# Guitaricet/relora

Hardware: NVIDIA H100
Metric: training throughput, llama ReLoRA (tokens/s, whole job, device-timed, max over ranks) (higher is better)
Workload: dtype bf16

## Files before the change

relora_b200/csrc/attention.cu:

```cuda
#include <cuda.h>

#include <cstdio>
#include <cstdlib>
#include <mutex>
#include <stdexcept>
#include <string>
#include <unordered_map>

#include "attention.h"
#include "common.cuh"
#include "sm90.cuh"
#include "tensormap.h"

namespace rb {

using namespace sm90;

namespace {

constexpr int BQ = 64;
constexpr int kPanel = 64 * 128;
constexpr int kThreads = 128;
constexpr int kMaxHeadDim = 256;
constexpr float kNegInf = -1e30f;

constexpr int smem_bytes(int nres, int np) { return (nres + 4) * np * kPanel + 1024 + 1024; }
constexpr int dq_out_panels(int np) { return np <= 3 ? np : 2; }
constexpr int dkv_out_panels(int np) { return np <= 2 ? np : 2; }
constexpr int splits(int np, int no) { return (np + no - 1) / no; }

__device__ __forceinline__ float fast_exp2(float x) {
  float y;
  asm("ex2.approx.ftz.f32 %0, %1;" : "=f"(y) : "f"(x));
  return y;
}

__device__ __forceinline__ void frag_to_a(const float (&d)[32], int kk, uint32_t (&a)[4]) {
  a[0] = pack_bf16x2(d[8 * kk + 0], d[8 * kk + 1]);
  a[1] = pack_bf16x2(d[8 * kk + 2], d[8 * kk + 3]);
  a[2] = pack_bf16x2(d[8 * kk + 4], d[8 * kk + 5]);
  a[3] = pack_bf16x2(d[8 * kk + 6], d[8 * kk + 7]);
}
template <int NSTEPS>
__device__ __forceinline__ void mma_steps_kk(float (&d)[32], uint32_t a, uint32_t b) {
#pragma unroll
  for (int ks = 0; ks < NSTEPS; ++ks) {
    const uint32_t ofs = (ks >> 2) * kPanel + (ks & 3) * 32;
    wgmma_bf16_ss_n64<0, 0>(d, desc_kmajor(a + ofs), desc_kmajor(b + ofs));
  }
}
template <int NP>
__device__ __forceinline__ void mma_tiles_kk(float (&d)[32], uint32_t a, uint32_t b, int nks) {
  if constexpr (NP == 1) {
    mma_steps_kk<4>(d, a, b);
  } else {
    switch (nks - 4 * (NP - 1)) {
      case 1: mma_steps_kk<4 * NP - 3>(d, a, b); break;
      case 2: mma_steps_kk<4 * NP - 2>(d, a, b); break;
      case 3: mma_steps_kk<4 * NP - 1>(d, a, b); break;
      default: mma_steps_kk<4 * NP>(d, a, b); break;
    }
  }
}
__device__ __forceinline__ void pack_a(const float (&p)[32], uint32_t (&a)[4][4]) {
#pragma unroll
  for (int kk = 0; kk < 4; ++kk) {
    frag_to_a(p, kk, a[kk]);
    fence_regs(a[kk]);
  }
}
template <int NO, int N = NO>
__device__ __forceinline__ void mma_regs_tile(float (&d)[NO][32], const uint32_t (&a)[4][4], uint32_t t, int nout) {
  if constexpr (N > 1) {
    if (nout < N) return mma_regs_tile<NO, N - 1>(d, a, t, nout);
  }
#pragma unroll
  for (int kk = 0; kk < 4; ++kk) {
#pragma unroll
    for (int j = 0; j < N; ++j) wgmma_bf16_rs_n64<1>(d[j], a[kk], desc_mnmajor(t + j * kPanel + kk * 2048));
  }
}
__device__ __forceinline__ void zero32(float (&d)[32]) {
#pragma unroll
  for (int i = 0; i < 32; ++i) d[i] = 0.f;
}

struct Smem {
  uint8_t* res[2];
  uint8_t* str[2][2];
  uint64_t* res_bar;
  uint64_t* str_bar;
  float* col_lse;
  float* col_delta;
};
template <int NRES, int NP>
__device__ __forceinline__ Smem smem_layout() {
  constexpr int kTile = NP * kPanel;
  extern __shared__ uint8_t smem_raw[];
  uint8_t* s = reinterpret_cast<uint8_t*>((reinterpret_cast<uintptr_t>(smem_raw) + 1023) & ~uintptr_t(1023));
  Smem m;
  m.res[0] = s;
  m.res[1] = s + (NRES - 1) * kTile;
  for (int b = 0; b < 2; ++b)
    for (int o = 0; o < 2; ++o) m.str[b][o] = s + (NRES + 2 * b + o) * kTile;
  m.res_bar = reinterpret_cast<uint64_t*>(s + (NRES + 4) * kTile);
  m.str_bar = m.res_bar + 1;
  m.col_lse = reinterpret_cast<float*>(s + (NRES + 4) * kTile + 64);
  m.col_delta = m.col_lse + 64;
  return m;
}
struct TileSrc {
  const CUtensorMap* map;
  int head;
};
template <int NP>
__device__ __forceinline__ void load_tile(TileSrc s, uint64_t* bar, uint8_t* dst, int row) {
#pragma unroll
  for (int pn = 0; pn < NP; ++pn) tma_load_3d(s.map, bar, dst + pn * kPanel, 64 * pn, s.head, row);
}
template <int NP>
__device__ __forceinline__ void issue_pair(const Smem& m, int buf, TileSrc s0, TileSrc s1, int row) {
  mbar_arrive_expect_tx(&m.str_bar[buf], 2 * NP * kPanel);
  load_tile<NP>(s0, &m.str_bar[buf], m.str[buf][0], row);
  load_tile<NP>(s1, &m.str_bar[buf], m.str[buf][1], row);
}
template <int NRES, int NP>
__device__ __forceinline__ void prologue(const Smem& m, TileSrc r0, TileSrc r1, int res_row, TileSrc s0, TileSrc s1, int row0, int nblk) {
  if (threadIdx.x == 0) {
    mbar_init(m.res_bar, 1);
    mbar_init(&m.str_bar[0], 1);
    mbar_init(&m.str_bar[1], 1);
    fence_barrier_init();
  }
  __syncthreads();
  pdl_wait();
  if (warp_id() == 0) {
    if (elect_one()) {
      mbar_arrive_expect_tx(m.res_bar, NRES * NP * kPanel);
      load_tile<NP>(r0, m.res_bar, m.res[0], res_row);
      if (NRES == 2) load_tile<NP>(r1, m.res_bar, m.res[1], res_row);
      for (int j = 0; j < 2 && j < nblk; ++j) issue_pair<NP>(m, j, s0, s1, row0 + j * BQ);
    }
    __syncwarp();
  }
  mbar_wait(m.res_bar, 0);
}

struct HeadMap {
  int hs, wk, wv, group;
  __device__ __forceinline__ int q(int h) const { return h * hs; }
  __device__ __forceinline__ int k(int kv) const { return kv * hs + wk; }
  __device__ __forceinline__ int v(int kv) const { return kv * hs + wv; }
};
struct FwdArgs {
  bf16* out;
  long long ld_out;
  float* lse;
  int B, T, nh, hd;
  float scale_log2;
  HeadMap hm;
};

template <int NP>
__global__ void __launch_bounds__(kThreads) attn_fwd_kernel(const __grid_constant__ CUtensorMap map_qkv, const FwdArgs p) {
  if (threadIdx.x == 0) pdl_launch_dependents();
  const int nqb = (p.T + BQ - 1) / BQ;
  const int qb = nqb - 1 - blockIdx.x;
  const int h = blockIdx.y, b = blockIdx.z;
  const int q0 = qb * BQ, rowbase = b * p.T;
  const int nkb = qb + 1;
  const int nks = (p.hd + 15) / 16;
  const Smem m = smem_layout<1, NP>();
  const int kv = h / p.hm.group;
  const int hq = p.hm.q(h), hk = p.hm.k(kv), hv = p.hm.v(kv);
  prologue<1, NP>(m, {&map_qkv, hq}, {&map_qkv, hq}, rowbase + q0, {&map_qkv, hk}, {&map_qkv, hv}, rowbase, nkb);
  const uint32_t sq = smem_u32(m.res[0]);
  float o[NP][32], mrow[2] = {kNegInf, kNegInf}, lrow[2] = {0.f, 0.f};
#pragma unroll
  for (int pn = 0; pn < NP; ++pn) zero32(o[pn]);
  const int r_lo = q0 + frag_row(0);
  for (int j = 0; j < nkb; ++j) {
    const int buf = j & 1;
    mbar_wait(&m.str_bar[buf], (j >> 1) & 1);
    float s[32];
    zero32(s);
    wgmma_fence();
    mma_tiles_kk<NP>(s, sq, smem_u32(m.str[buf][0]), nks);
    wgmma_commit();
    wgmma_wait<0>();
    fence_regs(s);
    float mx[2] = {mrow[0], mrow[1]};
#pragma unroll
    for (int i = 0; i < 32; ++i) {
      const int hr = (i >> 1) & 1;
      float v = s[i] * p.scale_log2;
      if (j == qb && j * BQ + frag_col(i) > r_lo + 8 * hr) v = kNegInf;
      s[i] = v;
      mx[hr] = fmaxf(mx[hr], v);
    }
#pragma unroll
    for (int hr = 0; hr < 2; ++hr) {
      mx[hr] = fmaxf(mx[hr], __shfl_xor_sync(0xffffffffu, mx[hr], 1));
      mx[hr] = fmaxf(mx[hr], __shfl_xor_sync(0xffffffffu, mx[hr], 2));
    }
    const float corr[2] = {fast_exp2(mrow[0] - mx[0]), fast_exp2(mrow[1] - mx[1])};
    float ls[2] = {0.f, 0.f};
#pragma unroll
    for (int i = 0; i < 32; ++i) {
      const int hr = (i >> 1) & 1;
      s[i] = fast_exp2(s[i] - mx[hr]);
      ls[hr] += s[i];
#pragma unroll
      for (int pn = 0; pn < NP; ++pn) o[pn][i] *= corr[hr];
    }
#pragma unroll
    for (int hr = 0; hr < 2; ++hr) {
      lrow[hr] = lrow[hr] * corr[hr] + ls[hr];
      mrow[hr] = mx[hr];
    }
    uint32_t pa[4][4];
    pack_a(s, pa);
#pragma unroll
    for (int pn = 0; pn < NP; ++pn) fence_regs(o[pn]);
    wgmma_fence();
    mma_regs_tile<NP>(o, pa, smem_u32(m.str[buf][1]), NP);
    wgmma_commit();
    wgmma_wait<0>();
#pragma unroll
    for (int pn = 0; pn < NP; ++pn) fence_regs(o[pn]);
    __syncthreads();
    if (warp_id() == 0 && j + 2 < nkb) {
      if (elect_one()) issue_pair<NP>(m, buf, {&map_qkv, hk}, {&map_qkv, hv}, rowbase + (j + 2) * BQ);
      __syncwarp();
    }
  }
#pragma unroll
  for (int hr = 0; hr < 2; ++hr) {
    lrow[hr] += __shfl_xor_sync(0xffffffffu, lrow[hr], 1);
    lrow[hr] += __shfl_xor_sync(0xffffffffu, lrow[hr], 2);
  }
#pragma unroll
  for (int pn = 0; pn < NP; ++pn) {
#pragma unroll
    for (int i = 0; i < 32; i += 2) {
      const int hr = (i >> 1) & 1;
      const int q = r_lo + 8 * hr, c = 64 * pn + frag_col(i);
      if (q >= p.T || c >= p.hd) continue;
      const float inv = 1.f / lrow[hr];
      *reinterpret_cast<uint32_t*>(p.out + (long long)(rowbase + q) * p.ld_out + h * p.hd + c) =
          pack_bf16x2(o[pn][i] * inv, o[pn][i + 1] * inv);
    }
  }
  if ((threadIdx.x & 3) == 0) {
#pragma unroll
    for (int hr = 0; hr < 2; ++hr) {
      const int q = r_lo + 8 * hr;
      if (q < p.T) p.lse[((long long)b * p.nh + h) * p.T + q] = mrow[hr] + __log2f(lrow[hr]);
    }
  }
}

__global__ void __launch_bounds__(256) attn_delta_kernel(const bf16* __restrict__ o, long long ld_o, const bf16* __restrict__ dout,
                                                         long long ld_do, float* __restrict__ delta, int B, int T, int nh, int hd) {
  pdl_wait();
  pdl_launch_dependents();
  const long long total = (long long)B * T * nh;
  for (long long i = blockIdx.x * (long long)blockDim.x + threadIdx.x; i < total; i += (long long)gridDim.x * blockDim.x) {
    const int h = int(i % nh);
    const long long row = i / nh;
    const bf16* a = o + row * ld_o + h * hd;
    const bf16* g = dout + row * ld_do + h * hd;
    float acc = 0.f;
    for (int q = 0; q < hd; q += 8) {
      float x[8], y[8];
      unpack8(*reinterpret_cast<const uint4*>(a + q), x);
      unpack8(*reinterpret_cast<const uint4*>(g + q), y);
#pragma unroll
      for (int j = 0; j < 8; ++j) acc += x[j] * y[j];
    }
    const long long bb = row / T, t = row % T;
    delta[(bb * nh + h) * T + t] = acc;
  }
}

struct BwdArgs {
  const float* lse;
  const float* delta;
  bf16* dqkv;
  long long ld_dqkv;
  int B, T, nh, hd;
  float scale, scale_log2;
  HeadMap hm;
};

__device__ __forceinline__ void store_rows(bf16* base, long long ld, int row0, int rows_valid, int col_ofs, int hd, const float (&d)[32], float sc) {
#pragma unroll
  for (int i = 0; i < 32; i += 2) {
    const int r = frag_row(i), c = frag_col(i);
    if (row0 + r >= rows_valid || c >= hd) continue;
    *reinterpret_cast<uint32_t*>(base + (long long)row0 * ld + (long long)r * ld + col_ofs + c) = pack_bf16x2(d[i] * sc, d[i + 1] * sc);
  }
}
template <int NO>
__device__ __forceinline__ void store_panels(bf16* base, long long ld, int row0, int rows_valid, int col_ofs, int hd, int pn0, int nout,
                                             const float (&d)[NO][32], float sc) {
#pragma unroll
  for (int j = 0; j < NO; ++j)
    if (j < nout) store_rows(base, ld, row0, rows_valid, col_ofs + 64 * (pn0 + j), hd - 64 * (pn0 + j), d[j], sc);
}

template <int NP>
__global__ void __launch_bounds__(kThreads) attn_bwd_dq_kernel(const __grid_constant__ CUtensorMap map_qkv,
                                                               const __grid_constant__ CUtensorMap map_do, const BwdArgs p) {
  constexpr int NO = dq_out_panels(NP), NSPLIT = splits(NP, dq_out_panels(NP));
  if (threadIdx.x == 0) pdl_launch_dependents();
  const int nqb = (p.T + BQ - 1) / BQ;
  const int qb = nqb - 1 - blockIdx.x / NSPLIT;
  const int pn0 = (blockIdx.x % NSPLIT) * NO;
  const int nout = NP % NO == 0 ? NO : min(NO, NP - pn0);
  const int h = blockIdx.y, b = blockIdx.z;
  const int q0 = qb * BQ, rowbase = b * p.T;
  const int nkb = qb + 1;
  const int nks = (p.hd + 15) / 16;
  const Smem m = smem_layout<2, NP>();
  const int kv = h / p.hm.group;
  const int hq = p.hm.q(h), hk = p.hm.k(kv), hv = p.hm.v(kv);
  prologue<2, NP>(m, {&map_qkv, hq}, {&map_do, h}, rowbase + q0, {&map_qkv, hk}, {&map_qkv, hv}, rowbase, nkb);
  const long long bh = (long long)b * p.nh + h;
  const int r_lo = q0 + frag_row(0);
  float lse[2], dlt[2];
#pragma unroll
  for (int hr = 0; hr < 2; ++hr) {
    const int q = min(r_lo + 8 * hr, p.T - 1);
    lse[hr] = p.lse[bh * p.T + q];
    dlt[hr] = p.delta[bh * p.T + q];
  }
  float dq[NO][32];
#pragma unroll
  for (int j = 0; j < NO; ++j) zero32(dq[j]);
  for (int j = 0; j < nkb; ++j) {
    const int buf = j & 1;
    mbar_wait(&m.str_bar[buf], (j >> 1) & 1);
    float s[32], dp[32];
    zero32(s);
    zero32(dp);
    wgmma_fence();
    mma_tiles_kk<NP>(s, smem_u32(m.res[0]), smem_u32(m.str[buf][0]), nks);
    mma_tiles_kk<NP>(dp, smem_u32(m.res[1]), smem_u32(m.str[buf][1]), nks);
    wgmma_commit();
    wgmma_wait<0>();
    fence_regs(s);
    fence_regs(dp);
#pragma unroll
    for (int i = 0; i < 32; ++i) {
      const int hr = (i >> 1) & 1;
      const bool ok = !(j == qb && j * BQ + frag_col(i) > r_lo + 8 * hr);
      const float pr = ok ? fast_exp2(s[i] * p.scale_log2 - lse[hr]) : 0.f;
      s[i] = pr * (dp[i] - dlt[hr]);
    }
    uint32_t pa[4][4];
    pack_a(s, pa);
    wgmma_fence();
    mma_regs_tile<NO>(dq, pa, smem_u32(m.str[buf][0]) + pn0 * kPanel, nout);
    wgmma_commit();
    wgmma_wait<0>();
#pragma unroll
    for (int jo = 0; jo < NO; ++jo) fence_regs(dq[jo]);
    __syncthreads();
    if (warp_id() == 0 && j + 2 < nkb) {
      if (elect_one()) issue_pair<NP>(m, buf, {&map_qkv, hk}, {&map_qkv, hv}, rowbase + (j + 2) * BQ);
      __syncwarp();
    }
  }
  store_panels<NO>(p.dqkv + (long long)rowbase * p.ld_dqkv, p.ld_dqkv, q0, p.T, hq * p.hd, p.hd, pn0, nout, dq, p.scale);
}

template <int NP>
__global__ void __launch_bounds__(kThreads) attn_bwd_dkv_kernel(const __grid_constant__ CUtensorMap map_qkv,
                                                                const __grid_constant__ CUtensorMap map_do, const BwdArgs p) {
  constexpr int NO = dkv_out_panels(NP), NSPLIT = splits(NP, dkv_out_panels(NP));
  if (threadIdx.x == 0) pdl_launch_dependents();
  const int nkb = (p.T + BQ - 1) / BQ;
  const int kb = blockIdx.x / NSPLIT;
  const int pn0 = (blockIdx.x % NSPLIT) * NO;
  const int nout = NP % NO == 0 ? NO : min(NO, NP - pn0);
  const int kv = blockIdx.y, b = blockIdx.z;
  const int k0 = kb * BQ, rowbase = b * p.T;
  const int nblk = nkb - kb;
  const int nks = (p.hd + 15) / 16;
  const Smem m = smem_layout<2, NP>();
  const int h0 = kv * p.hm.group;
  prologue<2, NP>(m, {&map_qkv, p.hm.k(kv)}, {&map_qkv, p.hm.v(kv)}, rowbase + k0, {&map_qkv, p.hm.q(h0)}, {&map_do, h0}, rowbase + k0, nblk);
  if (nblk == 1 && p.hm.group > 1 && warp_id() == 0) {
    if (elect_one()) issue_pair<NP>(m, 1, {&map_qkv, p.hm.q(h0 + 1)}, {&map_do, h0 + 1}, rowbase + k0);
    __syncwarp();
  }
  const int key_lo = k0 + frag_row(0);
  float dk[NO][32], dv[NO][32];
#pragma unroll
  for (int j = 0; j < NO; ++j) {
    zero32(dk[j]);
    zero32(dv[j]);
  }
  int hg = h0, qs = k0;
  for (int jj = 0; hg < ((int)blockIdx.y + 1) * p.hm.group; ++jj) {
    const int buf = jj & 1;
    const long long bh = (long long)b * p.nh + hg;
    if (threadIdx.x < BQ) {
      const int qc = min(qs + (int)threadIdx.x, p.T - 1);
      m.col_lse[threadIdx.x] = p.lse[bh * p.T + qc];
      m.col_delta[threadIdx.x] = p.delta[bh * p.T + qc];
    }
    __syncthreads();
    mbar_wait(&m.str_bar[buf], (jj >> 1) & 1);
    float st[32], dpt[32];
    zero32(st);
    zero32(dpt);
    wgmma_fence();
    mma_tiles_kk<NP>(st, smem_u32(m.res[0]), smem_u32(m.str[buf][0]), nks);
    mma_tiles_kk<NP>(dpt, smem_u32(m.res[1]), smem_u32(m.str[buf][1]), nks);
    wgmma_commit();
    wgmma_wait<0>();
    fence_regs(st);
    fence_regs(dpt);
#pragma unroll
    for (int i = 0; i < 32; ++i) {
      const int q = qs + frag_col(i), key = key_lo + 8 * ((i >> 1) & 1);
      const bool ok = q < p.T && key <= q;
      const float pr = ok ? fast_exp2(st[i] * p.scale_log2 - m.col_lse[frag_col(i)]) : 0.f;
      dpt[i] = pr * (dpt[i] - m.col_delta[frag_col(i)]);
      st[i] = pr;
    }
    uint32_t pa[4][4], dsa[4][4];
    pack_a(st, pa);
    pack_a(dpt, dsa);
    wgmma_fence();
    mma_regs_tile<NO>(dv, pa, smem_u32(m.str[buf][1]) + pn0 * kPanel, nout);
    mma_regs_tile<NO>(dk, dsa, smem_u32(m.str[buf][0]) + pn0 * kPanel, nout);
    wgmma_commit();
    wgmma_wait<0>();
#pragma unroll
    for (int j = 0; j < NO; ++j) {
      fence_regs(dv[j]);
      fence_regs(dk[j]);
    }
    __syncthreads();
    if (warp_id() == 0) {
      int h2 = hg, q2 = qs + 2 * BQ;
      while (q2 >= p.T) {
        q2 -= nkb * BQ - k0;
        ++h2;
      }
      if (h2 < ((int)blockIdx.y + 1) * p.hm.group) {
        if (elect_one()) issue_pair<NP>(m, buf, {&map_qkv, p.hm.q(h2)}, {&map_do, h2}, rowbase + q2);
        __syncwarp();
      }
    }
    qs += BQ;
    if (qs >= p.T) {
      qs = k0;
      ++hg;
    }
  }
  bf16* base = p.dqkv + (long long)rowbase * p.ld_dqkv;
  store_panels<NO>(base, p.ld_dqkv, k0, p.T, p.hm.k(blockIdx.y) * p.hd, p.hd, pn0, nout, dk, p.scale);
  store_panels<NO>(base, p.ld_dqkv, k0, p.T, p.hm.v(blockIdx.y) * p.hd, p.hd, pn0, nout, dv, 1.0f);
}

struct HeadMapKey {
  const void* ptr;
  long long ld, rows;
  int hd, heads;
  bool operator==(const HeadMapKey& o) const { return ptr == o.ptr && ld == o.ld && rows == o.rows && hd == o.hd && heads == o.heads; }
};
struct HeadMapHash {
  size_t operator()(const HeadMapKey& k) const {
    size_t h = reinterpret_cast<size_t>(k.ptr);
    h ^= std::hash<long long>()(k.ld * 1315423911ll + k.rows) + 0x9e3779b97f4a7c15ull + (h << 6) + (h >> 2);
    h ^= std::hash<long long>()(((long long)k.hd << 32) | (unsigned)k.heads) + 0x9e3779b97f4a7c15ull + (h << 6) + (h >> 2);
    return h;
  }
};
std::unordered_map<HeadMapKey, CUtensorMap, HeadMapHash> g_head_maps;
std::mutex g_head_maps_mu;

CUtensorMap head_map(const void* ptr, long long ld, long long rows, int hd, int heads) {
  HeadMapKey key{ptr, ld, rows, hd, heads};
  {
    std::lock_guard<std::mutex> lk(g_head_maps_mu);
    auto it = g_head_maps.find(key);
    if (it != g_head_maps.end()) return it->second;
  }
  CUtensorMap m = make_map_3d_bf16(ptr, hd, heads, rows, hd, ld, 64, 1, 64);
  std::lock_guard<std::mutex> lk(g_head_maps_mu);
  if (g_head_maps.size() > 4096) g_head_maps.clear();
  g_head_maps.emplace(key, m);
  return m;
}

void check_shape(int B, int T, int nh, int nkv, int hd, bool interleaved) {
  if (B <= 0 || T <= 0 || nh <= 0) throw std::runtime_error("attention: empty problem");
  if (hd <= 0 || hd % 8 != 0 || hd > kMaxHeadDim)
    throw std::runtime_error("attention: head_dim must be a multiple of 8 and <= 256, got " + std::to_string(hd));
  if (nkv <= 0 || nh % nkv != 0)
    throw std::runtime_error("attention: nh (" + std::to_string(nh) + ") must be a multiple of nkv (" + std::to_string(nkv) + ")");
  if (interleaved && nkv != nh) throw std::runtime_error("attention: the interleaved qkv layout has no grouped-query form (nkv must equal nh)");
}

HeadMap head_map_of(int nh, int nkv, bool interleaved) {
  return interleaved ? HeadMap{3, 1, 2, 1} : HeadMap{1, nh, nh + nkv, nh / nkv};
}

template <int NP>
void fwd_np(const AttnDesc& d, const CUtensorMap& map, cudaStream_t stream) {
  constexpr int smem = smem_bytes(1, NP);
  static const bool configured =
      (check(cudaFuncSetAttribute(attn_fwd_kernel<NP>, cudaFuncAttributeMaxDynamicSharedMemorySize, smem), "cudaFuncSetAttribute(attn_fwd)"), true);
  (void)configured;
  FwdArgs p;
  p.out = reinterpret_cast<bf16*>(d.out); p.ld_out = d.ld_out; p.lse = d.lse;
  p.B = d.B; p.T = d.T; p.nh = d.nh; p.hd = d.hd;
  p.scale_log2 = d.scale * 1.4426950408889634f;
  p.hm = head_map_of(d.nh, d.nkv, d.interleaved);
  const dim3 grid((unsigned)((d.T + BQ - 1) / BQ), (unsigned)d.nh, (unsigned)d.B);
  launch_k(attn_fwd_kernel<NP>, grid, kThreads, smem, stream, map, p);
  RB_CHECK_LAUNCH("attn_fwd_kernel");
}

template <int NP>
void bwd_np(const AttnBwdDesc& d, const CUtensorMap& map_qkv, const CUtensorMap& map_do, cudaStream_t stream) {
  constexpr int smem = smem_bytes(2, NP);
  static const bool configured =
      (check(cudaFuncSetAttribute(attn_bwd_dq_kernel<NP>, cudaFuncAttributeMaxDynamicSharedMemorySize, smem), "cudaFuncSetAttribute(attn_dq)"),
       check(cudaFuncSetAttribute(attn_bwd_dkv_kernel<NP>, cudaFuncAttributeMaxDynamicSharedMemorySize, smem), "cudaFuncSetAttribute(attn_dkv)"),
       true);
  (void)configured;
  BwdArgs p;
  p.lse = d.lse; p.delta = d.delta; p.dqkv = reinterpret_cast<bf16*>(d.dqkv); p.ld_dqkv = d.ld_dqkv;
  p.B = d.B; p.T = d.T; p.nh = d.nh; p.hd = d.hd;
  p.scale = d.scale; p.scale_log2 = d.scale * 1.4426950408889634f;
  p.hm = head_map_of(d.nh, d.nkv, d.interleaved);
  const unsigned nblk = (unsigned)((d.T + BQ - 1) / BQ);
  const dim3 grid_dkv(nblk * splits(NP, dkv_out_panels(NP)), (unsigned)d.nkv, (unsigned)d.B);
  launch_k(attn_bwd_dkv_kernel<NP>, grid_dkv, kThreads, smem, stream, map_qkv, map_do, p);
  RB_CHECK_LAUNCH("attn_bwd_dkv_kernel");
  const dim3 grid_dq(nblk * splits(NP, dq_out_panels(NP)), (unsigned)d.nh, (unsigned)d.B);
  launch_k(attn_bwd_dq_kernel<NP>, grid_dq, kThreads, smem, stream, map_qkv, map_do, p);
  RB_CHECK_LAUNCH("attn_bwd_dq_kernel");
}

int panels(int hd) { return (hd + 63) / 64; }

}

void attention_fwd(const AttnDesc& d, cudaStream_t stream) {
  check_shape(d.B, d.T, d.nh, d.nkv, d.hd, d.interleaved);
  const long long rows = (long long)d.B * d.T;
  CUtensorMap map = head_map(d.qkv, d.ld_qkv, rows, d.hd, d.nh + 2 * d.nkv);
  switch (panels(d.hd)) {
    case 1: fwd_np<1>(d, map, stream); break;
    case 2: fwd_np<2>(d, map, stream); break;
    case 3: fwd_np<3>(d, map, stream); break;
    default: fwd_np<4>(d, map, stream); break;
  }
}

void attention_bwd(const AttnBwdDesc& d, cudaStream_t stream) {
  check_shape(d.B, d.T, d.nh, d.nkv, d.hd, d.interleaved);
  const long long rows = (long long)d.B * d.T;
  CUtensorMap map_qkv = head_map(d.qkv, d.ld_qkv, rows, d.hd, d.nh + 2 * d.nkv);
  CUtensorMap map_do = head_map(d.dout, d.ld_dout, rows, d.hd, d.nh);
  {
    const long long total = rows * d.nh;
    const int grid = (int)std::min<long long>((total + 255) / 256, (long long)num_sms() * 8);
    launch_k(attn_delta_kernel, grid, 256, 0, stream, reinterpret_cast<const bf16*>(d.out), d.ld_out, reinterpret_cast<const bf16*>(d.dout),
             d.ld_dout, d.delta, d.B, d.T, d.nh, d.hd);
    RB_CHECK_LAUNCH("attn_delta_kernel");
  }
  switch (panels(d.hd)) {
    case 1: bwd_np<1>(d, map_qkv, map_do, stream); break;
    case 2: bwd_np<2>(d, map_qkv, map_do, stream); break;
    case 3: bwd_np<3>(d, map_qkv, map_do, stream); break;
    default: bwd_np<4>(d, map_qkv, map_do, stream); break;
  }
}

int attention_smem_bytes(int hd) { return smem_bytes(2, panels(hd)); }

long long attention_ds_pitch(int T) { return ((long long)T + 63) / 64 * 64; }
long long attention_ds_workspace_elems(int B, int T, int nh) {
  const long long Tp = attention_ds_pitch(T);
  return (long long)B * nh * Tp * Tp;
}

}
```

Before: 214,400.

## Coalesce delta kernel loads and overlap LSE/delta fetches with TMA waits

Rewrites the attention backward delta kernel so each warp cooperatively loads 32 (row, head) dot products with coalesced 16-byte loads, stages them in swizzled shared memory, and then has each lane reduce one row. The mbarrier wait on the resident Q/K/V tiles moves out of the prologue into each kernel, so LSE and delta loads overlap the TMA transfers. The dK/dV kernel also prefetches the next block's LSE/delta into registers during the current block. The delta path is a small share of the step, and the extra shared staging adds some complexity.

```diff
diff --git a/relora_b200/csrc/attention.cu b/relora_b200/csrc/attention.cu
--- a/relora_b200/csrc/attention.cu
+++ b/relora_b200/csrc/attention.cu
@@ -143,7 +143,6 @@
     }
     __syncwarp();
   }
-  mbar_wait(m.res_bar, 0);
 }
 
 struct HeadMap {
@@ -174,6 +173,7 @@
   const int kv = h / p.hm.group;
   const int hq = p.hm.q(h), hk = p.hm.k(kv), hv = p.hm.v(kv);
   prologue<1, NP>(m, {&map_qkv, hq}, {&map_qkv, hq}, rowbase + q0, {&map_qkv, hk}, {&map_qkv, hv}, rowbase, nkb);
+  mbar_wait(m.res_bar, 0);
   const uint32_t sq = smem_u32(m.res[0]);
   float o[NP][32], mrow[2] = {kNegInf, kNegInf}, lrow[2] = {0.f, 0.f};
 #pragma unroll
@@ -260,26 +260,57 @@
   }
 }
 
-__global__ void __launch_bounds__(256) attn_delta_kernel(const bf16* __restrict__ o, long long ld_o, const bf16* __restrict__ dout,
-                                                         long long ld_do, float* __restrict__ delta, int B, int T, int nh, int hd) {
+constexpr int kDeltaWarps = 4;
+constexpr int kDeltaChunks = 8;
+__global__ void __launch_bounds__(kDeltaWarps * 32) attn_delta_kernel(const bf16* __restrict__ o, long long ld_o, const bf16* __restrict__ dout,
+                                                                       long long ld_do, float* __restrict__ delta, int B, int T, int nh, int hd) {
+  __shared__ uint4 stage[kDeltaWarps][2][32][kDeltaChunks];
   pdl_wait();
   pdl_launch_dependents();
   const long long total = (long long)B * T * nh;
-  for (long long i = blockIdx.x * (long long)blockDim.x + threadIdx.x; i < total; i += (long long)gridDim.x * blockDim.x) {
-    const int h = int(i % nh);
-    const long long row = i / nh;
-    const bf16* a = o + row * ld_o + h * hd;
-    const bf16* g = dout + row * ld_do + h * hd;
+  const int lane = threadIdx.x & 31, w = threadIdx.x >> 5;
+  const int cpr = hd / 8;
+  for (long long s0 = ((long long)blockIdx.x * kDeltaWarps + w) * 32; s0 < total; s0 += (long long)gridDim.x * kDeltaWarps * 32) {
+    const long long row0 = s0 / nh;
+    const int h0 = int(s0 - row0 * nh);
     float acc = 0.f;
-    for (int q = 0; q < hd; q += 8) {
-      float x[8], y[8];
-      unpack8(*reinterpret_cast<const uint4*>(a + q), x);
-      unpack8(*reinterpret_cast<const uint4*>(g + q), y);
-#pragma unroll
-      for (int j = 0; j < 8; ++j) acc += x[j] * y[j];
-    }
-    const long long bb = row / T, t = row % T;
-    delta[(bb * nh + h) * T + t] = acc;
+    for (int c0 = 0; c0 < cpr; c0 += kDeltaChunks) {
+      const int nc = min(kDeltaChunks, cpr - c0);
+      uint4 xr[kDeltaChunks], yr[kDeltaChunks];
+#pragma unroll
+      for (int r = 0; r < kDeltaChunks; ++r) {
+        const int k = lane + 32 * r, ls = k / nc, c = k - ls * nc;
+        if (r < nc && s0 + ls < total) {
+          const int hh = h0 + ls;
+          const long long row = row0 + hh / nh;
+          const int col = (hh % nh) * hd + 8 * (c0 + c);
+          xr[r] = *reinterpret_cast<const uint4*>(o + row * ld_o + col);
+          yr[r] = *reinterpret_cast<const uint4*>(dout + row * ld_do + col);
+        }
+      }
+#pragma unroll
+      for (int r = 0; r < kDeltaChunks; ++r) {
+        const int k = lane + 32 * r, ls = k / nc, c = k - ls * nc;
+        if (r < nc && s0 + ls < total) {
+          stage[w][0][ls][c ^ (ls & 7)] = xr[r];
+          stage[w][1][ls][c ^ (ls & 7)] = yr[r];
+        }
+      }
+      __syncwarp();
+      for (int c = 0; c < nc; ++c) {
+        float x[8], y[8];
+        unpack8(stage[w][0][lane][c ^ (lane & 7)], x);
+        unpack8(stage[w][1][lane][c ^ (lane & 7)], y);
+#pragma unroll
+        for (int j = 0; j < 8; ++j) acc += x[j] * y[j];
+      }
+      __syncwarp();
+    }
+    if (s0 + lane < total) {
+      const int hh = h0 + lane;
+      const long long row = row0 + hh / nh, bb = row / T, t = row % T;
+      delta[(bb * nh + hh % nh) * T + t] = acc;
+    }
   }
 }
 
@@ -335,6 +366,7 @@
     lse[hr] = p.lse[bh * p.T + q];
     dlt[hr] = p.delta[bh * p.T + q];
   }
+  mbar_wait(m.res_bar, 0);
   float dq[NO][32];
 #pragma unroll
   for (int j = 0; j < NO; ++j) zero32(dq[j]);
@@ -403,13 +435,28 @@
     zero32(dv[j]);
   }
   int hg = h0, qs = k0;
+  float nlse = 0.f, ndlt = 0.f;
+  if (threadIdx.x < BQ) {
+    const long long i0 = ((long long)b * p.nh + h0) * p.T + min(k0 + (int)threadIdx.x, p.T - 1);
+    nlse = p.lse[i0];
+    ndlt = p.delta[i0];
+  }
+  mbar_wait(m.res_bar, 0);
   for (int jj = 0; hg < ((int)blockIdx.y + 1) * p.hm.group; ++jj) {
     const int buf = jj & 1;
-    const long long bh = (long long)b * p.nh + hg;
     if (threadIdx.x < BQ) {
-      const int qc = min(qs + (int)threadIdx.x, p.T - 1);
-      m.col_lse[threadIdx.x] = p.lse[bh * p.T + qc];
-      m.col_delta[threadIdx.x] = p.delta[bh * p.T + qc];
+      m.col_lse[threadIdx.x] = nlse;
+      m.col_delta[threadIdx.x] = ndlt;
+      int h1 = hg, q1 = qs + BQ;
+      if (q1 >= p.T) {
+        q1 = k0;
+        ++h1;
+      }
+      if (h1 < ((int)blockIdx.y + 1) * p.hm.group) {
+        const long long i1 = ((long long)b * p.nh + h1) * p.T + min(q1 + (int)threadIdx.x, p.T - 1);
+        nlse = p.lse[i1];
+        ndlt = p.delta[i1];
+      }
     }
     __syncthreads();
     mbar_wait(&m.str_bar[buf], (jj >> 1) & 1);
@@ -571,9 +618,9 @@
   CUtensorMap map_qkv = head_map(d.qkv, d.ld_qkv, rows, d.hd, d.nh + 2 * d.nkv);
   CUtensorMap map_do = head_map(d.dout, d.ld_dout, rows, d.hd, d.nh);
   {
-    const long long total = rows * d.nh;
-    const int grid = (int)std::min<long long>((total + 255) / 256, (long long)num_sms() * 8);
-    launch_k(attn_delta_kernel, grid, 256, 0, stream, reinterpret_cast<const bf16*>(d.out), d.ld_out, reinterpret_cast<const bf16*>(d.dout),
+    const long long warps = (rows * d.nh + 31) / 32;
+    const int grid = (int)std::min<long long>((warps + kDeltaWarps - 1) / kDeltaWarps, (long long)num_sms() * 8);
+    launch_k(attn_delta_kernel, grid, kDeltaWarps * 32, 0, stream, reinterpret_cast<const bf16*>(d.out), d.ld_out, reinterpret_cast<const bf16*>(d.dout),
              d.ld_dout, d.delta, d.B, d.T, d.nh, d.hd);
     RB_CHECK_LAUNCH("attn_delta_kernel");
   }
```

New measurement: 219,300 (median of 6 runs). 1.02x the previous value.
